# titoeb/RecModel

Hardware: AMD Instinct MI355X
Metric: ALS user+item row-updates/sec (higher is better)
Workload: dtype f32; 1 GPU; cfg3: WMF k=128+bias, 10000000x1000000 CSR, 99990947 nnz, alpha-log confidence, gamma=0.1, zipf_a=0.0; n_items=1000000, nnz=99990947, k=128, bias=True

## Files before the change

### recmodel_amd/csrc/wmf_dense.hip

```cpp
#include "wmf_common.h"
#include "wmf_internal.h"

#include <type_traits>
#include <utility>

template <int NFB, int NSPLIT, int S>
__device__ __forceinline__ void gram_body(const float* __restrict__ Y, int64_t m, int f, int ld, int bias,
                                          float* __restrict__ partial, int64_t step_lo, int64_t step_hi) {
    constexpr int NT = NFB * (NFB + 1) / 2;
    constexpr int NACC = (NT + NSPLIT - 1) / NSPLIT;
    const int lane = threadIdx.x & 63;
    const int r = lane & 15, q = lane >> 4;
    f32x4 acc[NACC];
#pragma unroll
    for (int i = 0; i < NACC; ++i) acc[i] = f32x4{0.f, 0.f, 0.f, 0.f};

    constexpr int U = 4;
    float cur[U][NFB], nxt[U][NFB];
    const int last_col = min(16 * (NFB - 1) + r, ld - 1);
    const float col_mask_last = (16 * (NFB - 1) + r < f) ? 1.f : 0.f;
    auto load_trip = [&](int64_t s0, float (&fr)[U][NFB]) {
#pragma unroll
        for (int uu = 0; uu < U; ++uu) {
            const int64_t row = min(4 * (s0 + uu) + q, m - 1);
            const float* yrow = Y + row * (int64_t)ld;
#pragma unroll
            for (int fb = 0; fb < NFB - 1; ++fb) fr[uu][fb] = yrow[16 * fb + r];
            fr[uu][NFB - 1] = yrow[last_col];
        }
    };
    if (step_lo < step_hi) load_trip(step_lo, cur);
    for (int64_t s0 = step_lo; s0 < step_hi; s0 += U) {
        if (s0 + U < step_hi) load_trip(s0 + U, nxt);
#pragma unroll
        for (int uu = 0; uu < U; ++uu) {
            const int64_t s = s0 + uu;
            const float rmask = (s < step_hi && 4 * s + q < m) ? 1.f : 0.f;
            float frag[NFB];
#pragma unroll
            for (int fb = 0; fb < NFB; ++fb) frag[fb] = cur[uu][fb] * rmask;
            frag[NFB - 1] *= col_mask_last;
            if (bias && r == 0) frag[0] = rmask;
            int t = 0;
#pragma unroll
            for (int bi = 0; bi < NFB; ++bi) {
#pragma unroll
                for (int bj = bi; bj < NFB; ++bj, ++t) {
                    if (t % NSPLIT == S) acc[t / NSPLIT] = WMF_MFMA16(frag[bi], frag[bj], acc[t / NSPLIT]);
                }
            }
        }
#pragma unroll
        for (int uu = 0; uu < U; ++uu)
#pragma unroll
            for (int fb = 0; fb < NFB; ++fb) cur[uu][fb] = nxt[uu][fb];
    }
    float* out = partial + (int64_t)blockIdx.x * NT * 256;
    int t = 0;
#pragma unroll
    for (int bi = 0; bi < NFB; ++bi) {
#pragma unroll
        for (int bj = bi; bj < NFB; ++bj, ++t) {
            if (t % NSPLIT == S) {
#pragma unroll
                for (int reg = 0; reg < 4; ++reg) out[(t * 4 + reg) * 64 + lane] = acc[t / NSPLIT][reg];
            }
        }
    }
}

typedef __bf16 gram_bf16x8 __attribute__((ext_vector_type(8)));
template <int NFB, bool AUG = false>
__device__ __forceinline__ void gram_body6(const float* __restrict__ Y, int64_t m, int f, int ld, int bias,
                                           float* __restrict__ partial, int64_t step_lo, int64_t step_hi) {
    constexpr int NT = NFB * (NFB + 1) / 2;
    constexpr int NG1 = (5 * NFB + 4) / 9;
    const int lane = threadIdx.x;
    const int r = lane & 15, q = lane >> 4;
    f32x4 acc[NT];
#pragma unroll
    for (int i = 0; i < NT; ++i) acc[i] = f32x4{0.f, 0.f, 0.f, 0.f};
    const int last_col = min(16 * (NFB - 1) + r, ld - 1);
    const float col_mask_last = (16 * (NFB - 1) + r < f) ? 1.f : 0.f;
    const bool bias_lane = bias && r == (AUG ? (f - 1) & 15 : 0);
    constexpr int ONE_FB = AUG ? NFB - 1 : 0;
    const int64_t stride = 32 * step_hi;
    auto load_blocks = [&](int64_t c0, float (&fr)[8][NFB], int fb_lo, int fb_hi) {
#pragma unroll
        for (int j = 0; j < 8; ++j) {
            const int64_t row = min(c0 + 8 * q + j, m - 1);
            const float* yrow = Y + row * (int64_t)ld;
#pragma unroll
            for (int fb = 0; fb < NFB; ++fb)
                if (fb >= fb_lo && fb < fb_hi) fr[j][fb] = yrow[fb == NFB - 1 ? last_col : 16 * fb + r];
        }
    };
    auto split = [&](int64_t c0, const float (&fr)[8][NFB], auto masked, gram_bf16x8 (&hi)[NFB], gram_bf16x8 (&mid)[NFB],
                     gram_bf16x8 (&lo)[NFB]) {
#pragma unroll
        for (int fb = 0; fb < NFB; ++fb) {
#pragma unroll
            for (int j = 0; j < 8; ++j) {
                const float rmask = (!decltype(masked)::value || c0 + 8 * q + j < m) ? 1.f : 0.f;
                float x = fr[j][fb];
                if (decltype(masked)::value) x *= rmask;
                if (fb == NFB - 1) x = AUG ? (col_mask_last != 0.f ? x : 0.f) : x * col_mask_last;
                if (fb == ONE_FB && bias_lane) x = rmask;
                const __bf16 h = (__bf16)x;
                const float r1 = x - (float)h;
                const __bf16 md = (__bf16)r1;
                hi[fb][j] = h; mid[fb][j] = md; lo[fb][j] = (__bf16)(r1 - (float)md);
            }
        }
    };
    auto products = [&](const gram_bf16x8 (&hi)[NFB], const gram_bf16x8 (&mid)[NFB], const gram_bf16x8 (&lo)[NFB]) {
        int t0 = 0;
#pragma unroll
        for (int bi = 0; bi < NFB; ++bi) {
#pragma unroll
            for (int bj = bi; bj < NFB; ++bj) acc[t0 + bj - bi] = __builtin_amdgcn_mfma_f32_16x16x32_bf16(lo[bi], hi[bj], acc[t0 + bj - bi], 0, 0, 0);
#pragma unroll
            for (int bj = bi; bj < NFB; ++bj) acc[t0 + bj - bi] = __builtin_amdgcn_mfma_f32_16x16x32_bf16(mid[bi], mid[bj], acc[t0 + bj - bi], 0, 0, 0);
#pragma unroll
            for (int bj = bi; bj < NFB; ++bj) acc[t0 + bj - bi] = __builtin_amdgcn_mfma_f32_16x16x32_bf16(hi[bi], lo[bj], acc[t0 + bj - bi], 0, 0, 0);
#pragma unroll
            for (int bj = bi; bj < NFB; ++bj) acc[t0 + bj - bi] = __builtin_amdgcn_mfma_f32_16x16x32_bf16(mid[bi], hi[bj], acc[t0 + bj - bi], 0, 0, 0);
#pragma unroll
            for (int bj = bi; bj < NFB; ++bj) acc[t0 + bj - bi] = __builtin_amdgcn_mfma_f32_16x16x32_bf16(hi[bi], mid[bj], acc[t0 + bj - bi], 0, 0, 0);
#pragma unroll
            for (int bj = bi; bj < NFB; ++bj) acc[t0 + bj - bi] = __builtin_amdgcn_mfma_f32_16x16x32_bf16(hi[bi], hi[bj], acc[t0 + bj - bi], 0, 0, 0);
            t0 += NFB - bi;
        }
    };
    float cur[8][NFB], nxt[8][NFB];
    int64_t c0 = 32 * step_lo;
    if (c0 < m) {
        load_blocks(c0, cur, 0, NFB);
        for (; c0 + stride < m; c0 += stride) {
            gram_bf16x8 hi[NFB], mid[NFB], lo[NFB];
            load_blocks(c0 + stride, nxt, 0, NG1);
            __builtin_amdgcn_sched_barrier(0);
            split(c0, cur, std::false_type{}, hi, mid, lo);
            __builtin_amdgcn_sched_barrier(0);
            load_blocks(c0 + stride, nxt, NG1, NFB);
            __builtin_amdgcn_sched_barrier(0);
            products(hi, mid, lo);
            __builtin_amdgcn_sched_barrier(0);
#pragma unroll
            for (int j = 0; j < 8; ++j)
#pragma unroll
                for (int fb = 0; fb < NFB; ++fb) cur[j][fb] = nxt[j][fb];
        }
        gram_bf16x8 hi[NFB], mid[NFB], lo[NFB];
        split(c0, cur, std::true_type{}, hi, mid, lo);
        products(hi, mid, lo);
    }
    float* out = partial + (int64_t)blockIdx.x * NT * 256;
#pragma unroll
    for (int t = 0; t < NT; ++t)
#pragma unroll
        for (int reg = 0; reg < 4; ++reg) out[(t * 4 + reg) * 64 + lane] = acc[t][reg];
}

template <int NFB>
__global__ __launch_bounds__(64) void gram6_kernel(const float* __restrict__ Y, int64_t m, int f, int ld, int bias,
                                                   float* __restrict__ partial, int64_t steps_per_wave) {
    gram_body6<NFB>(Y, m, f, ld, bias, partial, blockIdx.x, gridDim.x);
}

template <int NFB>
__global__ __launch_bounds__(64) void gram6_aug_kernel(const float* __restrict__ g, int64_t m, int f1, int ld, int bias,
                                                       float* __restrict__ partial) {
    gram_body6<NFB, true>(g, m, f1, ld, bias, partial, blockIdx.x, gridDim.x);
}

template <int NFB, int NSPLIT>
__global__ __launch_bounds__(NSPLIT == 1 ? 64 : 256) void gram_kernel(const float* __restrict__ Y, int64_t m, int f, int ld, int bias,
                                                  float* __restrict__ partial, int64_t steps_per_wave) {
    const int64_t nsteps = (m + 3) / 4;
    int64_t lo = (int64_t)blockIdx.x * steps_per_wave;
    int64_t hi = lo + steps_per_wave;
    if (hi > nsteps) hi = nsteps;
    if (lo > hi) lo = hi;
    if constexpr (NSPLIT == 1) {
        gram_body<NFB, 1, 0>(Y, m, f, ld, bias, partial, lo, hi);
    } else {
        switch (__builtin_amdgcn_readfirstlane(threadIdx.x >> 6)) {
            case 0: gram_body<NFB, NSPLIT, 0>(Y, m, f, ld, bias, partial, lo, hi); break;
            case 1: gram_body<NFB, NSPLIT, 1>(Y, m, f, ld, bias, partial, lo, hi); break;
            case 2: gram_body<NFB, NSPLIT, 2>(Y, m, f, ld, bias, partial, lo, hi); break;
            default: gram_body<NFB, NSPLIT, 3>(Y, m, f, ld, bias, partial, lo, hi); break;
        }
    }
}

#define WMF_GRAM_SLICES 32
__global__ __launch_bounds__(256) void gram_reduce1_kernel(const float* __restrict__ partial, int nwaves, int f, int nfb,
                                                           double* __restrict__ slices) {
    const int e = blockIdx.x * blockDim.x + threadIdx.x;
    if (e >= f * f) return;
    int i = e / f, j = e % f;
    if (i > j) { int tmp = i; i = j; j = tmp; }
    const int bi = i >> 4, bj = j >> 4, ri = i & 15, cj = j & 15;
    const int t = bi * nfb - (bi * (bi - 1)) / 2 + (bj - bi);
    const int lane = cj + 16 * (ri >> 2), reg = ri & 3;
    const int nt = nfb * (nfb + 1) / 2;
    const float* p = partial + ((int64_t)t * 4 + reg) * 64 + lane;
    const int per = (nwaves + WMF_GRAM_SLICES - 1) / WMF_GRAM_SLICES;
    const int w0 = blockIdx.y * per, w1 = min(nwaves, w0 + per);
    double s = 0.0;
    for (int w = w0; w < w1; ++w) s += (double)p[(int64_t)w * nt * 256];
    slices[(int64_t)blockIdx.y * f * f + e] = s;
}

__global__ __launch_bounds__(256) void gram_reduce2_kernel(const double* __restrict__ slices, int f, double* __restrict__ G) {
    const int e = blockIdx.x * blockDim.x + threadIdx.x;
    if (e >= f * f) return;
    double s = 0.0;
#pragma unroll 8
    for (int k = 0; k < WMF_GRAM_SLICES; ++k) s += slices[(int64_t)k * f * f + e];
    G[e] = s;
}

template <int NFB>
static int launch_gram_nfb(const float* Y, int64_t m, int f, int ld, int bias, float* partial, int nwaves,
                           hipStream_t st) {
    const int64_t nsteps = (m + 3) / 4;
    const int64_t spw = (nsteps + nwaves - 1) / nwaves;
    if constexpr (NFB >= 7 && NFB <= 9) {
        if (!(wmf_debug_flags & WMF_DBG_F32_GRAM)) {
            static const char* nm = wmf_kname("gram6_kernel<%d>", NFB);
            WMF_LAUNCH(nm, (gram6_kernel<NFB>), dim3(nwaves), dim3(64), 0, st, Y, m, f, ld, bias, partial, spw);
            return WMF_L_OK;
        }
    }
    if constexpr (NFB <= 9) {
        static const char* nm = wmf_kname("gram_kernel<%d, 1>", NFB);
        WMF_LAUNCH(nm, (gram_kernel<NFB, 1>), dim3(nwaves), dim3(64), 0, st, Y, m, f, ld, bias, partial, spw);
    } else {
        static const char* nm = wmf_kname("gram_kernel<%d, 4>", NFB);
        WMF_LAUNCH(nm, (gram_kernel<NFB, 4>), dim3(nwaves), dim3(256), 0, st, Y, m, f, ld, bias, partial, spw);
    }
    return WMF_L_OK;
}

int wmf_gram_max_waves(int f) {
    const int64_t nfb = (f + 15) / 16, nt = nfb * (nfb + 1) / 2;
    int64_t cap = ((int64_t)64 << 20) / (nt * 1024);
    if (cap > WMF_GRAM_MAX_WAVES) cap = WMF_GRAM_MAX_WAVES;
    return (int)(cap < 64 ? 64 : cap);
}

int wmf_gram_nwaves(int64_t m, int f) {
    int64_t nsteps = (m + 3) / 4;
    int64_t want = (nsteps + 31) / 32;
    if (want < 1) want = 1;
    const int cap = wmf_gram_max_waves(f);
    if (want > cap) want = cap;
    if (want > 1024) want -= want % 1024;
    return (int)want;
}

int wmf_launch_gram(const float* Y, int64_t m, int f, int ld, int bias, double* G_sum, float* partial, double* slices,
                    hipStream_t st) {
    if (m <= 0) return hipMemsetAsync(G_sum, 0, (size_t)f * f * sizeof(double), st) == hipSuccess ? WMF_L_OK : WMF_L_NO_KERNEL;
    const int nfb = (f + 15) / 16;
    const int nwaves = wmf_gram_nwaves(m, f);
    if (const int rc = wmf_dispatch_nfb<1, 17>(nfb, [&](auto n) { return launch_gram_nfb<decltype(n)::value>(Y, m, f, ld, bias, partial, nwaves, st); })) return rc;
    WMF_LAUNCH("gram_reduce1_kernel", gram_reduce1_kernel, dim3((f * f + 255) / 256, WMF_GRAM_SLICES), dim3(256), 0, st, partial,
               nwaves, f, nfb, slices);
    WMF_LAUNCH("gram_reduce2_kernel", gram_reduce2_kernel, dim3((f * f + 255) / 256), dim3(256), 0, st, slices, f, G_sum);
    return WMF_L_OK;
}

int wmf_launch_gram_aug(const float* g, int64_t m, int f, int ld, int bias, double* G_aug, float* partial, double* slices,
                        hipStream_t st) {
    const int f1 = f + (bias ? 1 : 0), nfb = (f1 + 15) / 16;
    if (nfb < 7 || nfb > 9) return WMF_L_NO_KERNEL;
    if (m <= 0) return hipMemsetAsync(G_aug, 0, (size_t)f1 * f1 * sizeof(double), st) == hipSuccess ? WMF_L_OK : WMF_L_NO_KERNEL;
    const int nwaves = wmf_gram_nwaves(m, f1);
    if (const int rc = wmf_dispatch_nfb<7, 9>(nfb, [&](auto n) {
            constexpr int NFB = decltype(n)::value;
            static const char* nm = wmf_kname("gram6_aug_kernel<%d>", NFB);
            WMF_LAUNCH(nm, (gram6_aug_kernel<NFB>), dim3(nwaves), dim3(64), 0, st, g, m, f1, ld, bias, partial);
            return (int)WMF_L_OK;
        })) return rc;
    WMF_LAUNCH("gram_reduce1_kernel", gram_reduce1_kernel, dim3((f1 * f1 + 255) / 256, WMF_GRAM_SLICES), dim3(256), 0, st, partial,
               nwaves, f1, nfb, slices);
    WMF_LAUNCH("gram_reduce2_kernel", gram_reduce2_kernel, dim3((f1 * f1 + 255) / 256), dim3(256), 0, st, slices, f1, G_aug);
    return WMF_L_OK;
}

__device__ __forceinline__ double rl_f64(double v, int lane) {
    const int lo = __builtin_amdgcn_readlane(__double2loint(v), lane);
    const int hi = __builtin_amdgcn_readlane(__double2hiint(v), lane);
    return __hiloint2double(hi, lo);
}

typedef double f64x4 __attribute__((ext_vector_type(4)));
#define WMF_MFMA16_F64(a, b, c) __builtin_amdgcn_mfma_f64_16x16x4f64((a), (b), (c), 0, 0, 0)
constexpr int FZ_LD = 66;

__device__ __forceinline__ f64x4 fz_mul_abt(const double* A, int la, const double* B, int lb, f64x4 c, int r, int q, double sign) {
#pragma unroll
    for (int kk = 0; kk < 4; ++kk) c = WMF_MFMA16_F64(sign * A[r * la + 4 * kk + q], B[r * lb + 4 * kk + q], c);
    return c;
}
__device__ __forceinline__ f64x4 fz_mul_ab(const double* A, int la, const double* B, int lb, f64x4 c, int r, int q, double sign) {
#pragma unroll
    for (int kk = 0; kk < 4; ++kk) c = WMF_MFMA16_F64(sign * A[r * la + 4 * kk + q], B[(4 * kk + q) * lb + r], c);
    return c;
}
__device__ __forceinline__ f64x4 fz_load(const double* T, int lt, int r, int q) {
    return f64x4{T[q * lt + r], T[(q + 4) * lt + r], T[(q + 8) * lt + r], T[(q + 12) * lt + r]};
}
__device__ __forceinline__ void fz_store(double* T, int lt, const f64x4& c, int r, int q) {
#pragma unroll
    for (int v = 0; v < 4; ++v) T[(q + 4 * v) * lt + r] = c[v];
}
__device__ __noinline__ int fz_diag(const double* D, double* Lt, double* Xt, int lt, int lane) {
    const int row = lane & 15;
    double a[16];
#pragma unroll
    for (int j = 0; j < 16; ++j) a[j] = D[row * lt + j];
    int fail = 0;
    double rinv[16];
#pragma unroll
    for (int K = 0; K < 16; ++K) {
        const double dk = rl_f64(a[K], K);
        if (!(dk > 0.0) && !fail) fail = K + 1;
        double y = __builtin_amdgcn_rsq(dk);
        y = y * (1.5 - 0.5 * dk * y * y);
        y = y * (1.5 - 0.5 * dk * y * y);
        rinv[K] = y;
        a[K] *= y;
#pragma unroll
        for (int j = K + 1; j < 16; ++j) a[j] -= a[K] * rl_f64(a[K], j);
    }
    double x[16];
#pragma unroll
    for (int i = 0; i < 16; ++i) {
        double sacc = (i == row) ? 1.0 : 0.0;
#pragma unroll
        for (int k = 0; k < i; ++k) sacc -= rl_f64(a[k], i) * x[k];
        x[i] = sacc * rinv[i];
    }
    if (lane < 16) {
#pragma unroll
        for (int j = 0; j < 16; ++j) {
            Lt[row * lt + j] = (j <= row) ? a[j] : 0.0;
            Xt[j * lt + row] = x[j];
        }
    }
    return fail;
}

__global__ __launch_bounds__(64, 1) void factorize64m_kernel(const double* __restrict__ G, int f, int ld, double lambda,
                                                             float* __restrict__ Wwhite, float* __restrict__ Wunwhite,
                                                             int32_t* __restrict__ info) {
    __shared__ __attribute__((aligned(16))) double Gs[64 * FZ_LD];
    __shared__ __attribute__((aligned(16))) double Xs[64 * FZ_LD];
    __shared__ __attribute__((aligned(16))) double Ts[16 * FZ_LD];
    const int lane = threadIdx.x, r = lane & 15, q = lane >> 4;
    const int nb = (f + 15) >> 4;
#pragma unroll 16
    for (int i = 0; i < 64; ++i) {
        const int j = lane;
        double v = (i == j) ? 1.0 : 0.0;
        const double gv = G[min(i, f - 1) * f + min(j, f - 1)];
        if (i < f && j < f) v = gv + (i == j ? lambda : 0.0);
        Gs[i * FZ_LD + j] = v;
        Xs[i * FZ_LD + j] = 0.0;
    }
    __builtin_amdgcn_fence(__ATOMIC_RELEASE, "wavefront");
    __builtin_amdgcn_wave_barrier();
    int fail = 0;
    auto tile = [&](double* M, int bi, int bj) { return M + (16 * bi) * FZ_LD + 16 * bj; };
    auto sync = [&]() { __builtin_amdgcn_fence(__ATOMIC_RELEASE, "wavefront"); __builtin_amdgcn_wave_barrier(); };
    for (int p = 0; p < nb; ++p) {
        const int bad = fz_diag(tile(Gs, p, p), tile(Gs, p, p), tile(Xs, p, p), FZ_LD, lane);
        if (bad && !fail) fail = 16 * p + bad;
        sync();
        for (int i = p + 1; i < nb; ++i) {
            const f64x4 c = fz_mul_abt(tile(Gs, i, p), FZ_LD, tile(Xs, p, p), FZ_LD, f64x4{0.0, 0.0, 0.0, 0.0}, r, q, 1.0);
            sync();
            fz_store(tile(Gs, i, p), FZ_LD, c, r, q);
            sync();
        }
        for (int i = p + 1; i < nb; ++i)
            for (int j = p + 1; j <= i; ++j) {
                const f64x4 c = fz_mul_abt(tile(Gs, i, p), FZ_LD, tile(Gs, j, p), FZ_LD, fz_load(tile(Gs, i, j), FZ_LD, r, q), r, q, -1.0);
                fz_store(tile(Gs, i, j), FZ_LD, c, r, q);
            }
        sync();
    }
    for (int p = 0; p < nb; ++p)
        for (int i = p + 1; i < nb; ++i) {
            f64x4 sacc = f64x4{0.0, 0.0, 0.0, 0.0};
            for (int k = p; k < i; ++k) sacc = fz_mul_ab(tile(Gs, i, k), FZ_LD, tile(Xs, k, p), FZ_LD, sacc, r, q, 1.0);
            fz_store(Ts, FZ_LD, sacc, r, q);
            sync();
            const f64x4 c = fz_mul_ab(tile(Xs, i, i), FZ_LD, Ts, FZ_LD, f64x4{0.0, 0.0, 0.0, 0.0}, r, q, -1.0);
            fz_store(tile(Xs, i, p), FZ_LD, c, r, q);
            sync();
        }
    const bool ok = fail == 0;
    if (lane == 0 && !ok) *info = fail;
#pragma unroll 8
    for (int i = 0; i < 64; ++i) {
        if (i >= f) break;
        for (int j = lane; j < ld; j += 64) {
            float wu = 0.f, ww = 0.f;
            if (j < f && ok) { wu = (float)Xs[i * FZ_LD + j]; ww = (float)Xs[j * FZ_LD + i]; }
            Wunwhite[i * ld + j] = wu;
            Wwhite[i * ld + j] = ww;
        }
    }
}

__host__ __device__ __forceinline__ int wmf_perm(int j, int f, int perm) {
    return perm == 0 ? j : perm == 1 ? (j == 0 ? 0 : f - j) : f - 1 - j;
}

__global__ __launch_bounds__(512, 1) void factorize_blocked_kernel(const double* __restrict__ G, int f, int ld, double lambda,
                                                                   float* __restrict__ Wwhite, float* __restrict__ Wunwhite,
                                                                   int32_t* __restrict__ info, double* __restrict__ work, int perm) {
    __shared__ __attribute__((aligned(16))) double Ts[8][16 * 18];
    __shared__ int bad;
    const int tid = threadIdx.x, lane = tid & 63, r = lane & 15, q = lane >> 4;
    const int wave = __builtin_amdgcn_readfirstlane(tid >> 6);
    const int nb = (f + 15) >> 4, fp = 16 * nb, LD = fp + 2;
    double* A = work;
    double* X = work + (size_t)fp * LD;
    if (tid == 0) bad = 0;
    for (int e = tid; e < fp * fp; e += 512) {
        const int i = e / fp, j = e % fp;
        double v = (i == j) ? 1.0 : 0.0;
        if (i < f && j < f) v = G[i * f + j] + (i == j ? lambda : 0.0);
        A[i * LD + j] = v;
        X[i * LD + j] = 0.0;
    }
    __syncthreads();
    auto tile = [&](double* M, int bi, int bj) { return M + (size_t)(16 * bi) * LD + 16 * bj; };
    for (int p = 0; p < nb; ++p) {
        if (wave == 0) {
            const int fail = fz_diag(tile(A, p, p), tile(A, p, p), tile(X, p, p), LD, lane);
            if (fail && lane == 0 && !bad) bad = 16 * p + fail;
        }
        __syncthreads();
        for (int i = p + 1 + wave; i < nb; i += 8) {
            const f64x4 c = fz_mul_abt(tile(A, i, p), LD, tile(X, p, p), LD, f64x4{0.0, 0.0, 0.0, 0.0}, r, q, 1.0);
            fz_store(tile(A, i, p), LD, c, r, q);
        }
        __syncthreads();
        int t = 0;
        for (int i = p + 1; i < nb; ++i)
            for (int j = p + 1; j <= i; ++j, ++t) {
                if ((t & 7) != wave) continue;
                const f64x4 c = fz_mul_abt(tile(A, i, p), LD, tile(A, j, p), LD, fz_load(tile(A, i, j), LD, r, q), r, q, -1.0);
                fz_store(tile(A, i, j), LD, c, r, q);
            }
        __syncthreads();
    }
    double* ts = Ts[wave];
    for (int p = wave; p < nb; p += 8)
        for (int i = p + 1; i < nb; ++i) {
            f64x4 sacc = f64x4{0.0, 0.0, 0.0, 0.0};
            for (int k = p; k < i; ++k) sacc = fz_mul_ab(tile(A, i, k), LD, tile(X, k, p), LD, sacc, r, q, 1.0);
            fz_store(ts, 18, sacc, r, q);
            __builtin_amdgcn_fence(__ATOMIC_RELEASE, "wavefront");
            __builtin_amdgcn_wave_barrier();
            const f64x4 c = fz_mul_ab(tile(X, i, i), LD, ts, 18, f64x4{0.0, 0.0, 0.0, 0.0}, r, q, -1.0);
            fz_store(tile(X, i, p), LD, c, r, q);
            __builtin_amdgcn_fence(__ATOMIC_RELEASE, "wavefront");
            __builtin_amdgcn_wave_barrier();
        }
    __syncthreads();
    const bool ok = bad == 0;
    if (tid == 0 && !ok) *info = bad;
    for (int e = tid; e < f * ld; e += 512) {
        const int i = e / ld, j = e % ld;
        float wu = 0.f, ww = 0.f;
        if (j < f && ok) { wu = (float)X[i * LD + wmf_perm(j, f, perm)]; ww = (float)X[j * LD + wmf_perm(i, f, perm)]; }
        Wunwhite[e] = wu;
        Wwhite[e] = ww;
    }
}

int wmf_launch_factorize(const double* G_sum, int f, int ld, double lambda, float* Wwhite, float* Wunwhite,
                         int32_t* info, double* gA, hipStream_t st, int perm) {
    if (f <= 64) {
        WmfProfScope ps("factorize64m_kernel", st);
        hipLaunchKernelGGL(factorize64m_kernel, dim3(1), dim3(64), 0, st, G_sum, f, ld, lambda, Wwhite, Wunwhite, info);
        return 0;
    }
    WmfProfScope ps("factorize_blocked_kernel", st);
    hipLaunchKernelGGL(factorize_blocked_kernel, dim3(1), dim3(512), 0, st, G_sum, f, ld, lambda, Wwhite, Wunwhite, info, gA, perm);
    return 0;
}

template <int NFB, bool W_IN_LDS, int NB0 = 0, int NBW = NFB>
__global__ __launch_bounds__(512) void transform_kernel(const float* __restrict__ in, int64_t m, int f, int ld,
                                                        const float* __restrict__ W, int set_col0_one,
                                                        float* __restrict__ out, float* __restrict__ col0_out,
                                                        int64_t nblocks16) {
    extern __shared__ __attribute__((aligned(16))) char smem_raw[];
    float* Wl = reinterpret_cast<float*>(smem_raw);
    constexpr int KP = 16 * NFB;
    constexpr int NP = 16 * NBW;
    constexpr int LDW = NP + 4;
    const int tid = threadIdx.x;
    __shared__ int nz[NFB * NBW];
    for (int e = tid; e < NFB * NBW; e += 512) nz[e] = 0;
    __syncthreads();
    for (int e = tid; e < KP * LDW; e += 512) {
        const int a = e / LDW, b = e % LDW, col = 16 * NB0 + b;
        const float v = (a < f && b < NP && col < f) ? W[a * ld + col] : 0.f;
        if constexpr (W_IN_LDS) Wl[e] = v;
        if (v != 0.f) nz[(a >> 4) * NBW + (b >> 4)] = 1;
    }
    __syncthreads();
    const int lane = tid & 63, wv = tid >> 6;
    const int r = lane & 15, q = lane >> 4;
    const int nch = ld >> 2;
    unsigned tmask[NFB];
#pragma unroll
    for (int t = 0; t < NFB; ++t) {
        unsigned mk = 0;
#pragma unroll
        for (int nb = 0; nb < NBW; ++nb) mk |= nz[t * NBW + nb] ? (1u << nb) : 0u;
        tmask[t] = __builtin_amdgcn_readfirstlane(mk);
    }
    constexpr bool DBL = NFB <= 11;
    const int64_t stride = (int64_t)gridDim.x * 8;
    auto request = [&](int64_t blk, float4 (&x)[NFB]) {
        const int64_t row = blk * 16 + r;
        const float4* irow = reinterpret_cast<const float4*>(in + (row < m ? row : 0) * (int64_t)ld);
#pragma unroll
        for (int t = 0; t < NFB; ++t) x[t] = irow[min(4 * t + q, nch - 1)];
    };
    auto block = [&](int64_t blk, float4 (&xc)[NFB], float4 (&xn)[NFB]) {
        if constexpr (DBL) { if (blk + stride < nblocks16) request(blk + stride, xn); }
        const int64_t row = blk * 16 + r;
        const bool rok = row < m;
        f32x4 acc[NBW];
#pragma unroll
        for (int nb = 0; nb < NBW; ++nb) acc[nb] = f32x4{0.f, 0.f, 0.f, 0.f};
#pragma unroll
        for (int t = 0; t < NFB; ++t) {
            const int c = 4 * t + q;
            const int k0 = 4 * c;
            float xe[4] = {xc[t].x, xc[t].y, xc[t].z, xc[t].w};
            if (t == NFB - 1) {
#pragma unroll
                for (int e = 0; e < 4; ++e) if (!(c < nch && k0 + e < f)) xe[e] = 0.f;
            }
            if (t == 0 && set_col0_one && q == 0) {
                if (rok && col0_out && NB0 == 0) col0_out[set_col0_one == 2 ? 2 * row + 1 : row] = xe[0];
                xe[0] = 1.f;
            }
            unsigned mv = tmask[t];
            asm volatile("" : "+v"(mv));
            const unsigned mk = __builtin_amdgcn_readfirstlane(mv);
#pragma unroll
            for (int nb = 0; nb < NBW; ++nb) {
                if (!(mk & (1u << nb))) continue;
#pragma unroll
                for (int e = 0; e < 4; ++e) {
                    const int k = k0 + e;
                    float b;
                    if constexpr (W_IN_LDS) {
                        b = Wl[k * LDW + 16 * nb + r];
                    } else {
                        const int col = 16 * (NB0 + nb) + r;
                        b = (k < f && col < f) ? W[k * ld + col] : 0.f;
                    }
                    acc[nb] = WMF_MFMA16(xe[e], b, acc[nb]);
                }
            }
        }
#pragma unroll
        for (int reg = 0; reg < 4; ++reg) {
            const int64_t orow = blk * 16 + 4 * q + reg;
            if (orow < m) {
                const bool sp = set_col0_one == 2;
                const int wid = sp ? f - 1 : ld;
                float* o = out + orow * (int64_t)wid;
#pragma unroll
                for (int nb = 0; nb < NBW; ++nb) {
                    const int col = 16 * (NB0 + nb) + r;
                    if (col < wid) o[col] = acc[nb][reg];
                    else if (sp && col == f - 1) col0_out[2 * orow] = acc[nb][reg];
                }
            }
        }
    };
    int64_t blk = (int64_t)blockIdx.x * 8 + wv;
    if constexpr (DBL) {
        float4 xa[NFB], xb[NFB];
        if (blk < nblocks16) request(blk, xa);
        while (blk < nblocks16) {
            block(blk, xa, xb);
            blk += stride;
            if (blk >= nblocks16) break;
            block(blk, xb, xa);
            blk += stride;
        }
    } else {
        float4 xa[NFB];
        for (; blk < nblocks16; blk += stride) {
            request(blk, xa);
            block(blk, xa, xa);
        }
    }
}

template <int NFB>
__global__ __launch_bounds__(512) void transform6_kernel(const float* __restrict__ in, int64_t m, int f, int ld,
                                                         const float* __restrict__ W, int set_col0_one,
                                                         float* __restrict__ out, float* __restrict__ col0_out,
                                                         int64_t nblocks16) {
    extern __shared__ __attribute__((aligned(16))) char smem_raw[];
    constexpr int NP = 16 * NFB;
    constexpr int NKC = (NP + 31) / 32;
    constexpr int KS = 176;
    static_assert(32 * NKC <= KS, "K does not fit the LDS row");
    __bf16* Wt = reinterpret_cast<__bf16*>(smem_raw);
    __shared__ int nz[NKC * NFB];
    const int tid = threadIdx.x;
    for (int e = tid; e < NKC * NFB; e += 512) nz[e] = 0;
    __syncthreads();
    const bool roll_n = set_col0_one == 3, roll_k = set_col0_one == 4;
    typedef __bf16 stage_bf16x8 __attribute__((ext_vector_type(8)));
    stage_bf16x8* Ws = reinterpret_cast<stage_bf16x8*>(Wt);
    for (int it = tid; it < NP * (KS / 8); it += 512) {
        const int k8 = it / NP, n = it - k8 * NP;
        const int rn = roll_n ? 1 : 0, rk = roll_k ? 1 : 0;
        const int ns = n + rn == f ? 0 : n + rn;
        float v[8];
#pragma unroll
        for (int j = 0; j < 8; ++j) {
            const int k = 8 * k8 + j;
            const int ks = k + rk == f ? 0 : k + rk;
            const bool in_w = k < f && n < f;
            v[j] = W[in_w ? ks * ld + ns : 0];
            if (!in_w) v[j] = 0.f;
        }
        stage_bf16x8 ph, pm, pl;
        bool any = false;
#pragma unroll
        for (int j = 0; j < 8; ++j) {
            const __bf16 h = (__bf16)v[j];
            const float r1 = v[j] - (float)h;
            const __bf16 md = (__bf16)r1;
            ph[j] = h; pm[j] = md; pl[j] = (__bf16)(r1 - (float)md);
            any |= v[j] != 0.f;
        }
        const int at = (n * KS + 8 * k8) / 8;
        Ws[at] = ph;
        Ws[NP * KS / 8 + at] = pm;
        Ws[2 * NP * KS / 8 + at] = pl;
        if (any) nz[(k8 >> 2) * NFB + (n >> 4)] = 1;
    }
    __syncthreads();
    const int lane = tid & 63, wv = __builtin_amdgcn_readfirstlane(tid >> 6);
    const int r = lane & 15, q = lane >> 4;
    const int nch = ld >> 2;
    unsigned cmask[NKC];
#pragma unroll
    for (int c = 0; c < NKC; ++c) {
        unsigned mk = 0;
#pragma unroll
        for (int nb = 0; nb < NFB; ++nb) mk |= nz[c * NFB + nb] ? (1u << nb) : 0u;
        cmask[c] = __builtin_amdgcn_readfirstlane(mk);
    }
    typedef __bf16 bf16x8_t __attribute__((ext_vector_type(8)));
    const bf16x8_t* Wl = reinterpret_cast<const bf16x8_t*>(Wt);
    const int64_t stride = (int64_t)gridDim.x * 8;
    auto request = [&](int64_t blk, float4 (&x)[2 * NKC]) {
        const int64_t row = blk * 16 + r;
        const float4* irow = reinterpret_cast<const float4*>(in + (row < m ? row : 0) * (int64_t)ld);
#pragma unroll
        for (int c = 0; c < NKC; ++c) {
            x[2 * c] = irow[min(8 * c + 2 * q, nch - 1)];
            x[2 * c + 1] = irow[min(8 * c + 2 * q + 1, nch - 1)];
        }
    };
    const bool in_one = set_col0_one >= 1 && set_col0_one <= 3;
    const bool sp = set_col0_one == 2 || set_col0_one == 3;
    auto block = [&](int64_t blk, float4 (&xc)[2 * NKC]) {
        const int64_t row = blk * 16 + r;
        const bool rok = row < m;
        float bias_of_row = 0.f;
        f32x4 acc[NFB];
#pragma unroll
        for (int nb = 0; nb < NFB; ++nb) acc[nb] = f32x4{0.f, 0.f, 0.f, 0.f};
#pragma unroll
        for (int c = 0; c < NKC; ++c) {
            const int k0 = 32 * c + 8 * q;
            float xe[8] = {xc[2 * c].x, xc[2 * c].y, xc[2 * c].z, xc[2 * c].w, xc[2 * c + 1].x, xc[2 * c + 1].y, xc[2 * c + 1].z, xc[2 * c + 1].w};
            if (32 * c + 32 > f) {
#pragma unroll
                for (int e = 0; e < 8; ++e) if (!(k0 + e < f)) xe[e] = 0.f;
            }
            if (c == 0 && in_one && q == 0) {
                if (rok && col0_out) col0_out[sp ? 2 * row + 1 : row] = xe[0];
                bias_of_row = xe[0];
                xe[0] = 1.f;
            }
            bf16x8_t ah, am, al;
#pragma unroll
            for (int e = 0; e < 8; ++e) {
                const __bf16 h = (__bf16)xe[e];
                const float r1 = xe[e] - (float)h;
                const __bf16 md = (__bf16)r1;
                ah[e] = h; am[e] = md; al[e] = (__bf16)(r1 - (float)md);
            }
            unsigned mv = cmask[c];
            asm volatile("" : "+v"(mv));
            const unsigned mk = __builtin_amdgcn_readfirstlane(mv);
#pragma unroll
            for (int nb = 0; nb < NFB; ++nb) {
                if (!(mk & (1u << nb))) continue;
                const int at = ((16 * nb + r) * KS + 32 * c + 8 * q) / 8;
                const bf16x8_t bh = Wl[at], bm = Wl[NP * KS / 8 + at], bl = Wl[2 * NP * KS / 8 + at];
                f32x4 cc = acc[nb];
                cc = __builtin_amdgcn_mfma_f32_16x16x32_bf16(al, bh, cc, 0, 0, 0);
                cc = __builtin_amdgcn_mfma_f32_16x16x32_bf16(am, bm, cc, 0, 0, 0);
                cc = __builtin_amdgcn_mfma_f32_16x16x32_bf16(ah, bl, cc, 0, 0, 0);
                cc = __builtin_amdgcn_mfma_f32_16x16x32_bf16(am, bh, cc, 0, 0, 0);
                cc = __builtin_amdgcn_mfma_f32_16x16x32_bf16(ah, bm, cc, 0, 0, 0);
                cc = __builtin_amdgcn_mfma_f32_16x16x32_bf16(ah, bh, cc, 0, 0, 0);
                acc[nb] = cc;
            }
        }
        const int wid = sp ? f - 1 : ld;
        const bool stuff = set_col0_one == 3 && (r & 7) < 2;
        const int stuff_sh = 2 * (r >> 3) + (r & 7);
        auto store_rows = [&](auto full) {
#pragma unroll
            for (int reg = 0; reg < 4; ++reg) {
                const int64_t orow = blk * 16 + 4 * q + reg;
                const unsigned bbits = set_col0_one == 3 ? (unsigned)__builtin_amdgcn_ds_bpermute((4 * q + reg) * 4, __builtin_bit_cast(int, bias_of_row)) : 0u;
                if (decltype(full)::value || orow < m) {
                    float* o = out + orow * (int64_t)wid;
#pragma unroll
                    for (int nb = 0; nb < NFB; ++nb) {
                        const int col = 16 * nb + r;
                        float v = acc[nb][reg];
                        if (16 * nb < 128) {
                            const unsigned vb = __builtin_bit_cast(unsigned, v);
                            v = __builtin_bit_cast(float, stuff ? ((vb & ~1u) | ((bbits >> (4 * nb + stuff_sh)) & 1u)) : vb);
                        }
                        if (nb < NFB - 1 || col < wid) o[col] = v;
                        else if (sp && col == f - 1) col0_out[2 * orow] = v;
                    }
                }
            }
        };
        if (blk * 16 + 16 <= m) store_rows(std::true_type{});
        else store_rows(std::false_type{});
    };
    float4 xa[2 * NKC];
    for (int64_t blk = (int64_t)blockIdx.x * 8 + wv; blk < nblocks16; blk += stride) {
        request(blk, xa);
        block(blk, xa);
    }
}

template <int NFB>
static void launch_transform6(const float* in, int64_t m, int f, int ld, const float* W, int set_col0_one, float* out,
                              float* col0_out, int64_t grid, int64_t nblk, hipStream_t st) {
    constexpr size_t lds = (size_t)3 * 16 * NFB * 176 * 2;
    static_assert(lds <= 158 * 1024, "W planes do not fit LDS");
    if (grid > wmf_cu_count()) grid = wmf_cu_count();
    static const char* nm = wmf_kname("transform6_kernel<%d>", NFB);
    WMF_LAUNCH_LDS(nm, (transform6_kernel<NFB>), lds, dim3((unsigned)grid), dim3(512), lds, st, in, m, f, ld, W, set_col0_one, out,
                   col0_out, nblk);
}

template <int NFB, int NB0, int NBW>
static void launch_transform_slice(const float* in, int64_t m, int f, int ld, const float* W, int set_col0_one, float* out,
                                   float* col0_out, int64_t grid, int64_t nblk, hipStream_t st) {
    constexpr size_t lds = (size_t)16 * NFB * (16 * NBW + 4) * 4;
    static_assert(lds <= 150 * 1024, "slice too wide");
    static const char* nm = wmf_kname("transform_kernel<%d, true, %d, %d>", NFB, NB0, NBW);
    WMF_LAUNCH_LDS(nm, (transform_kernel<NFB, true, NB0, NBW>), lds, dim3((unsigned)grid), dim3(512), lds, st, in, m, f, ld, W,
                   set_col0_one, out, col0_out, nblk);
}

template <int NFB>
static int launch_transform_nfb(const float* in, int64_t m, int f, int ld, const float* W, int set_col0_one, float* out,
                                 float* col0_out, hipStream_t st) {
    constexpr int KP = 16 * NFB, LDW = KP + 4;
    constexpr size_t lds = (size_t)KP * LDW * 4;
    const int64_t nblk = (m + 15) / 16;
    int64_t grid = (nblk + 7) / 8;
    if (grid > 1024) grid = 1024;
    if (grid < 1) grid = 1;
    constexpr bool WIDE = NFB >= 7 && NFB <= 9;
// ... 304 lines not shown
```

Baseline: 463.4 million row-updates/s.

## Keep Cholesky factorization in LDS and vectorize Gram reduce over upper tiles

Adds an LDS-resident path for the blocked Cholesky/inverse factorization when the factor dimension fits in ten 16-blocks. The packed lower-triangular tiles and diagonal inverses live in shared memory instead of global scratch, and the triangular-inverse sweep keeps intermediate tiles in registers. Separately, the first Gram reduction now reads float4 partials only for upper-triangle tiles, unrolls by 8, and writes both symmetric entries. The aim is to cut global-memory latency in the serial single-block factorization and redundant partial reads in the reduction, at the cost of a large dynamic-LDS allocation and more complex indexing.

Result: no change. 465.6 million row-updates/s, median of 4 (+0.5%).

```diff
diff --git a/recmodel_amd/csrc/wmf_dense.hip b/recmodel_amd/csrc/wmf_dense.hip
--- a/recmodel_amd/csrc/wmf_dense.hip
+++ b/recmodel_amd/csrc/wmf_dense.hip
@@ -197,20 +197,38 @@
 #define WMF_GRAM_SLICES 32
 __global__ __launch_bounds__(256) void gram_reduce1_kernel(const float* __restrict__ partial, int nwaves, int f, int nfb,
                                                            double* __restrict__ slices) {
-    const int e = blockIdx.x * blockDim.x + threadIdx.x;
-    if (e >= f * f) return;
-    int i = e / f, j = e % f;
-    if (i > j) { int tmp = i; i = j; j = tmp; }
-    const int bi = i >> 4, bj = j >> 4, ri = i & 15, cj = j & 15;
-    const int t = bi * nfb - (bi * (bi - 1)) / 2 + (bj - bi);
-    const int lane = cj + 16 * (ri >> 2), reg = ri & 3;
     const int nt = nfb * (nfb + 1) / 2;
-    const float* p = partial + ((int64_t)t * 4 + reg) * 64 + lane;
+    const int x4 = blockIdx.x * blockDim.x + threadIdx.x;
+    if (x4 >= nt * 64) return;
+    int t = x4 >> 6, bi = 0;
+    while (t >= nfb - bi) { t -= nfb - bi; ++bi; }
+    const int bj = bi + t, reg = (x4 >> 4) & 3, lane = 4 * (x4 & 15);
+    const int i = 16 * bi + 4 * (lane >> 4) + reg, j0 = 16 * bj + (lane & 15);
+    const float4* p = reinterpret_cast<const float4*>(partial) + x4;
+    const int64_t stride = (int64_t)nt * 64;
     const int per = (nwaves + WMF_GRAM_SLICES - 1) / WMF_GRAM_SLICES;
     const int w0 = blockIdx.y * per, w1 = min(nwaves, w0 + per);
-    double s = 0.0;
-    for (int w = w0; w < w1; ++w) s += (double)p[(int64_t)w * nt * 256];
-    slices[(int64_t)blockIdx.y * f * f + e] = s;
+    double s[4] = {0.0, 0.0, 0.0, 0.0};
+    int w = w0;
+    for (; w + 8 <= w1; w += 8) {
+        float4 v[8];
+#pragma unroll
+        for (int u = 0; u < 8; ++u) v[u] = p[(w + u) * stride];
+#pragma unroll
+        for (int u = 0; u < 8; ++u) { s[0] += (double)v[u].x; s[1] += (double)v[u].y; s[2] += (double)v[u].z; s[3] += (double)v[u].w; }
+    }
+    for (; w < w1; ++w) {
+        const float4 v = p[w * stride];
+        s[0] += (double)v.x; s[1] += (double)v.y; s[2] += (double)v.z; s[3] += (double)v.w;
+    }
+    double* out = slices + (int64_t)blockIdx.y * f * f;
+#pragma unroll
+    for (int c = 0; c < 4; ++c) {
+        const int j = j0 + c;
+        if (i >= f || j >= f || i > j) continue;
+        out[i * f + j] = s[c];
+        out[j * f + i] = s[c];
+    }
 }
 
 __global__ __launch_bounds__(256) void gram_reduce2_kernel(const double* __restrict__ slices, int f, double* __restrict__ G) {
@@ -267,8 +285,8 @@
     const int nfb = (f + 15) / 16;
     const int nwaves = wmf_gram_nwaves(m, f);
     if (const int rc = wmf_dispatch_nfb<1, 17>(nfb, [&](auto n) { return launch_gram_nfb<decltype(n)::value>(Y, m, f, ld, bias, partial, nwaves, st); })) return rc;
-    WMF_LAUNCH("gram_reduce1_kernel", gram_reduce1_kernel, dim3((f * f + 255) / 256, WMF_GRAM_SLICES), dim3(256), 0, st, partial,
-               nwaves, f, nfb, slices);
+    WMF_LAUNCH("gram_reduce1_kernel", gram_reduce1_kernel, dim3((nfb * (nfb + 1) / 2 * 64 + 255) / 256, WMF_GRAM_SLICES), dim3(256), 0, st,
+               partial, nwaves, f, nfb, slices);
     WMF_LAUNCH("gram_reduce2_kernel", gram_reduce2_kernel, dim3((f * f + 255) / 256), dim3(256), 0, st, slices, f, G_sum);
     return WMF_L_OK;
 }
@@ -285,8 +303,8 @@
             WMF_LAUNCH(nm, (gram6_aug_kernel<NFB>), dim3(nwaves), dim3(64), 0, st, g, m, f1, ld, bias, partial);
             return (int)WMF_L_OK;
         })) return rc;
-    WMF_LAUNCH("gram_reduce1_kernel", gram_reduce1_kernel, dim3((f1 * f1 + 255) / 256, WMF_GRAM_SLICES), dim3(256), 0, st, partial,
-               nwaves, f1, nfb, slices);
+    WMF_LAUNCH("gram_reduce1_kernel", gram_reduce1_kernel, dim3((nfb * (nfb + 1) / 2 * 64 + 255) / 256, WMF_GRAM_SLICES), dim3(256), 0, st,
+               partial, nwaves, f1, nfb, slices);
     WMF_LAUNCH("gram_reduce2_kernel", gram_reduce2_kernel, dim3((f1 * f1 + 255) / 256), dim3(256), 0, st, slices, f1, G_aug);
     return WMF_L_OK;
 }
@@ -422,9 +440,133 @@
     return perm == 0 ? j : perm == 1 ? (j == 0 ? 0 : f - j) : f - 1 - j;
 }
 
+constexpr int FZ_LDS_NB = 10;
+constexpr int FZ_TS = 17;
+constexpr int FZ_TILE = 16 * FZ_TS;
+static inline size_t fz_lds_bytes(int nb) { return (size_t)(nb * (nb + 1) / 2 + nb) * FZ_TILE * sizeof(double); }
+
+__device__ __forceinline__ f64x4 fz_mul_ab_reg(const double* A, int la, const f64x4& b, f64x4 c, int r, int q, double sign) {
+#pragma unroll
+    for (int kk = 0; kk < 4; ++kk) c = WMF_MFMA16_F64(sign * A[r * la + 4 * kk + q], b[kk], c);
+    return c;
+}
+
+__device__ __forceinline__ void factorize_lds_body(const double* __restrict__ G, int f, int ld, double lambda,
+                                                   float* __restrict__ Wwhite, float* __restrict__ Wunwhite,
+                                                   int32_t* __restrict__ info, double* __restrict__ work, int perm, double* Ls) {
+    __shared__ int bad;
+    const int tid = threadIdx.x, lane = tid & 63, r = lane & 15, q = lane >> 4;
+    const int wave = __builtin_amdgcn_readfirstlane(tid >> 6);
+    const int nb = (f + 15) >> 4, fp = 16 * nb, LD = fp + 2;
+    double* Xd = Ls + (nb * (nb + 1) / 2) * FZ_TILE;
+    double* X = work + (size_t)fp * LD;
+    auto tile = [&](int bi, int bj) { return Ls + (bi * (bi + 1) / 2 + bj) * FZ_TILE; };
+    if (tid == 0) bad = 0;
+    const int nel = (nb * (nb + 1) / 2) * 256;
+    for (int e0 = tid; e0 < nel; e0 += 8 * 512) {
+        double gv[8];
+        int at[8];
+#pragma unroll
+        for (int u = 0; u < 8; ++u) {
+            const int e = min(e0 + u * 512, nel - 1);
+            int t = e >> 8, bi = 0;
+            while (t > bi) { ++bi; t -= bi; }
+            const int i = 16 * bi + ((e >> 4) & 15), j = 16 * t + (e & 15);
+            gv[u] = G[min(i, f - 1) * f + min(j, f - 1)];
+            at[u] = (i < f && j < f ? 0 : 2) | (i == j ? 1 : 0) | ((e >> 8) * FZ_TILE + ((e >> 4) & 15) * FZ_TS + (e & 15)) << 2;
+        }
+#pragma unroll
+        for (int u = 0; u < 8; ++u) {
+            double v = (at[u] & 1) ? 1.0 : 0.0;
+            if (!(at[u] & 2)) v = gv[u] + ((at[u] & 1) ? lambda : 0.0);
+            Ls[at[u] >> 2] = v;
+        }
+    }
+    __syncthreads();
+    auto diag = [&](int p) {
+        const int fail = fz_diag(tile(p, p), tile(p, p), Xd + p * FZ_TILE, FZ_TS, lane);
+        if (fail && lane == 0 && !bad) bad = 16 * p + fail;
+    };
+    if (wave == 0) diag(0);
+    __syncthreads();
+    for (int p = 0; p + 1 < nb; ++p) {
+        for (int i = p + 1 + wave; i < nb; i += 8) {
+            const f64x4 c = fz_mul_abt(tile(i, p), FZ_TS, Xd + p * FZ_TILE, FZ_TS, f64x4{0.0, 0.0, 0.0, 0.0}, r, q, 1.0);
+            fz_store(tile(i, p), FZ_TS, c, r, q);
+        }
+        __syncthreads();
+        auto trail = [&](int i, int j) {
+            const f64x4 c = fz_mul_abt(tile(i, p), FZ_TS, tile(j, p), FZ_TS, fz_load(tile(i, j), FZ_TS, r, q), r, q, -1.0);
+            fz_store(tile(i, j), FZ_TS, c, r, q);
+        };
+        if (wave == 0) {
+            trail(p + 1, p + 1);
+            __builtin_amdgcn_fence(__ATOMIC_RELEASE, "wavefront");
+            __builtin_amdgcn_wave_barrier();
+            diag(p + 1);
+        } else {
+            int t = 0;
+            for (int i = p + 2; i < nb; ++i)
+                for (int j = p + 1; j <= i; ++j, ++t)
+                    if (t % 7 + 1 == wave) trail(i, j);
+        }
+        __syncthreads();
+    }
+    for (int p = wave; p + 1 < nb; p += 8) {
+        f64x4 xc[FZ_LDS_NB];
+        xc[0] = fz_load(Xd + p * FZ_TILE, FZ_TS, r, q);
+#pragma unroll
+        for (int d = 1; d < FZ_LDS_NB; ++d) {
+            const int i = p + d;
+            if (i < nb) {
+                f64x4 sacc = f64x4{0.0, 0.0, 0.0, 0.0};
+#pragma unroll
+                for (int k = 0; k < d; ++k) sacc = fz_mul_ab_reg(tile(i, p + k), FZ_TS, xc[k], sacc, r, q, 1.0);
+                xc[d] = fz_mul_ab_reg(Xd + i * FZ_TILE, FZ_TS, sacc, f64x4{0.0, 0.0, 0.0, 0.0}, r, q, -1.0);
+                fz_store(X + (size_t)(16 * i) * LD + 16 * p, LD, xc[d], r, q);
+            }
+        }
+    }
+    __syncthreads();
+    const bool ok = bad == 0;
+    if (tid == 0 && !ok) *info = bad;
+    struct XRef { int lds, glb, sel; };
+    auto xref = [&](int i, int j) {
+        const int bi = i >> 4, bj = j >> 4;
+        return XRef{bi * FZ_TILE + (i & 15) * FZ_TS + (j & 15), i * LD + j, bi < bj ? 0 : bi == bj ? 1 : 2};
+    };
+    for (int e0 = tid; e0 < f * ld; e0 += 4 * 512) {
+        double ul[4], ug[4], wl[4], wg[4];
+        int su[4], sw[4];
+#pragma unroll
+        for (int u = 0; u < 4; ++u) {
+            const int e = min(e0 + u * 512, f * ld - 1);
+            const int i = e / ld, j = min(e % ld, f - 1);
+            const XRef a = xref(i, wmf_perm(j, f, perm)), b = xref(j, wmf_perm(i, f, perm));
+            ul[u] = Xd[a.lds]; ug[u] = X[a.glb]; su[u] = a.sel;
+            wl[u] = Xd[b.lds]; wg[u] = X[b.glb]; sw[u] = b.sel;
+        }
+        asm volatile("" : "+v"(ul[0]), "+v"(ul[1]), "+v"(ul[2]), "+v"(ul[3]), "+v"(ug[0]), "+v"(ug[1]), "+v"(ug[2]), "+v"(ug[3]),
+                          "+v"(wl[0]), "+v"(wl[1]), "+v"(wl[2]), "+v"(wl[3]), "+v"(wg[0]), "+v"(wg[1]), "+v"(wg[2]), "+v"(wg[3]));
+#pragma unroll
+        for (int u = 0; u < 4; ++u) {
+            const int e = e0 + u * 512;
+            if (e >= f * ld) break;
+            const bool live = e % ld < f && ok;
+            Wunwhite[e] = live ? (float)(su[u] == 0 ? 0.0 : su[u] == 1 ? ul[u] : ug[u]) : 0.f;
+            Wwhite[e] = live ? (float)(sw[u] == 0 ? 0.0 : sw[u] == 1 ? wl[u] : wg[u]) : 0.f;
+        }
+    }
+}
+
 __global__ __launch_bounds__(512, 1) void factorize_blocked_kernel(const double* __restrict__ G, int f, int ld, double lambda,
                                                                    float* __restrict__ Wwhite, float* __restrict__ Wunwhite,
                                                                    int32_t* __restrict__ info, double* __restrict__ work, int perm) {
+    extern __shared__ __attribute__((aligned(16))) double fz_dyn[];
+    if (((f + 15) >> 4) <= FZ_LDS_NB) {
+        factorize_lds_body(G, f, ld, lambda, Wwhite, Wunwhite, info, work, perm, fz_dyn);
+        return;
+    }
     __shared__ __attribute__((aligned(16))) double Ts[8][16 * 18];
     __shared__ int bad;
     const int tid = threadIdx.x, lane = tid & 63, r = lane & 15, q = lane >> 4;
@@ -494,8 +636,11 @@
         hipLaunchKernelGGL(factorize64m_kernel, dim3(1), dim3(64), 0, st, G_sum, f, ld, lambda, Wwhite, Wunwhite, info);
         return 0;
     }
+    const int nb = (f + 15) >> 4;
+    const size_t lds = nb <= FZ_LDS_NB ? fz_lds_bytes(nb) : 0;
+    WMF_LDS_CEILING(factorize_blocked_kernel, fz_lds_bytes(FZ_LDS_NB));
     WmfProfScope ps("factorize_blocked_kernel", st);
-    hipLaunchKernelGGL(factorize_blocked_kernel, dim3(1), dim3(512), 0, st, G_sum, f, ld, lambda, Wwhite, Wunwhite, info, gA, perm);
+    hipLaunchKernelGGL(factorize_blocked_kernel, dim3(1), dim3(512), lds, st, G_sum, f, ld, lambda, Wwhite, Wunwhite, info, gA, perm);
     return 0;
 }
 
```
